# raynbowy23/RegT-GCN

Measured on AMD Instinct MI355X. Metric: training steps/sec (graph-snapshots/sec), higher is better.
Workload: dtype fp32; 1 GPU; cfg3: ONE synthetic regional graph, 100000 nodes / 1000000 edges / 8 regions, F=32, T=12, O=1, hidden=256; RegionalTemporalGCN forward+MSE+backward per snapshot, RMSprop step once per K steps (run.py semantics); gemm_arithmetic=fp32 MFMA (v_mfma_f32_32x32x2_f32), global_nodes=100000, global_edges=1000000, global_regions=8, parallelism=single GPU

## Files before the change

### regt-gcn_amd/csrc/gemm.hip

```cpp
#include "kernels.h"
#include "gemm_fast.h"
#include "gemm_split.h"
#include "gemm_small.h"

namespace regt {

#ifdef REGT_WG_TRACE
__device__ long g_wg_trace[4 * WG_TRACE_MAX];
__device__ long g_wg_marks[8 * WG_TRACE_MAX];
#define WG_TRACE_T(name) const long name = wall_clock64()
#define WG_TRACE_END(N, ta, tb)                                                                                              \
    if (threadIdx.x == 0 && WG_TILE_ID < WG_TRACE_MAX && (N) == REGT_WG_TRACE_N) {                                            \
        long* q_ = g_wg_trace + 4L * WG_TILE_ID;                                                                              \
        q_[0] = ta; q_[1] = tb; q_[2] = wall_clock64();                                                                       \
        q_[3] = ((long)__builtin_amdgcn_s_getreg((31 << 11) | 4)) | ((long)__builtin_amdgcn_s_getreg((31 << 11) | 20) << 32); \
    }
#else
#define WG_TRACE_T(name)
#define WG_TRACE_END(N, ta, tb)
#endif

__device__ __forceinline__ float fast_sigmoid(float x) { return __builtin_amdgcn_rcpf(1.0f + __expf(-x)); }
__device__ __forceinline__ float fast_tanh(float x) { return 1.0f - 2.0f * __builtin_amdgcn_rcpf(1.0f + __expf(2.0f * x)); }
__device__ __forceinline__ float4 ld4(const float* p) { return *reinterpret_cast<const float4*>(p); }
// ... 122 lines not shown
        long node = m / e.T;
        int t = (int)(m - node * e.T);
        float hv = e.h[m * e.C + c];
        float Z = e.ZR[m * (2L * e.C) + c];
        float R = e.ZR[m * (2L * e.C) + e.C + c];
        e.dzr[m * (2L * e.C) + e.C + c] = cb_drp(v, hv, R);
        e.dh[m * e.C + c] = cb_dh(v, R, e.probs[t], e.dOH[node * e.C + c], Z);
    }
    static constexpr int ROUND_ROWS = 8;
    struct Aux { float4 h, Z, R, d; float p; };
    __device__ __forceinline__ Aux load(long m, int c) const {
        const long node = m / e.T;
        Aux a;
        a.p = e.probs[(int)(m - node * e.T)];
        a.h = ld4(e.h + m * e.C + c);
        a.Z = ld4(e.ZR + m * (2L * e.C) + c);
        a.R = ld4(e.ZR + m * (2L * e.C) + e.C + c);
        a.d = ld4(e.dOH + node * e.C + c);
        return a;
    }
    __device__ __forceinline__ void apply(long m, int c, float4 v, const Aux& a) const {
#define F_(k) cb_drp(v.k, a.h.k, a.R.k)
        if (e.dzr_bf16) st4_bf16(e.dzr, m * (2L * e.C) + e.C + c, REGT_V4(F_));
        else st4(e.dzr + m * (2L * e.C) + e.C + c, REGT_V4(F_));
#undef F_
#define F_(k) cb_dh(v.k, a.R.k, a.p, a.d.k, a.Z.k)
        st4(e.dh + m * e.C + c, REGT_V4(F_));
#undef F_
    }
    static constexpr int NVAR = 2;
    static constexpr bool HAS_ROWTAB = true;
    struct Col {};
    struct Tile { __amdgpu_buffer_rsrc_t h, zr, d, dzr, dh; int vc, vzr, sc, szr, vd, vdzr, sdzr, rstep; const EpiRowEnt* rt; };
    __device__ __forceinline__ int variant(int) const { return e.dzr_bf16 ? 1 : 0; }
    __device__ __forceinline__ EpiRowEnt vrow(long m) const {
        const long node = m / e.T;
        return EpiRowEnt{(int)(node * e.C * 4), e.probs[(int)(m - node * e.T)]};
    }
    template <int V> __device__ __forceinline__ Col vcol(int) const { return Col{}; }
    template <int V> __device__ __forceinline__ Tile vtile(const EpiGeom& g) const {
        Tile t;
        t.h = buf_srd(e.h + g.m0 * e.C + g.n0);
        t.dh = buf_srd(e.dh + g.m0 * e.C + g.n0);
        t.zr = buf_srd(e.ZR + g.m0 * (2L * e.C) + g.n0);
        t.d = buf_srd(e.dOH + g.n0);
        const long o = g.m0 * (2L * e.C) + e.C + g.n0;
        t.dzr = buf_srd((V & 1) ? reinterpret_cast<const char*>(e.dzr) + 2 * o : reinterpret_cast<const char*>(e.dzr) + 4 * o);
        t.vc = (g.rr * e.C + g.c) * 4;
        t.sc = g.step * e.C * 4;
        t.vzr = 2 * t.vc - g.c * 4;
        t.szr = 2 * t.sc;
        t.vd = g.c * 4;
        t.vdzr = (V & 1) ? t.vzr >> 1 : t.vzr;
        t.sdzr = (V & 1) ? t.szr >> 1 : t.szr;
        t.rt = g.rowtab + g.rr;
        t.rstep = g.step;
        return t;
    }
    struct VAux { float4 h, Z, R, d; float p; };
    template <int V> __device__ __forceinline__ VAux vload(const Tile& t, int i) const {
        const EpiRowEnt re = t.rt[i * t.rstep];
        VAux a;
        a.p = re.p;
        a.h = buf_ld4(t.h, t.vc, i * t.sc);
        a.Z = buf_ld4(t.zr, t.vzr, i * t.szr);
        a.R = buf_ld4(t.zr, t.vzr, i * t.szr + e.C * 4);
        a.d = buf_ld4(t.d, t.vd + re.off, 0);
        return a;
    }
    template <int V> __device__ __forceinline__ void vapply(const Tile& t, int i, float4 v, const Col&, const VAux& a) const {
#define F_(k) cb_drp(v.k, a.h.k, a.R.k)
        if (V & 1) buf_st4_bf16(t.dzr, t.vdzr + i * t.sdzr, 0, REGT_V4(F_));
        else buf_st4(t.dzr, t.vdzr + i * t.sdzr, 0, REGT_V4(F_));
#undef F_
#define F_(k) cb_dh(v.k, a.R.k, a.p, a.d.k, a.Z.k)
        buf_st4(t.dh, t.vc + i * t.sc, 0, REGT_V4(F_));
#undef F_
    }
};
struct EpiDgrad1GenF {
    EpiDgrad1 e;
    int parts;
    static constexpr int ROUND_ROWS = 8;
    __device__ __forceinline__ static float half_wave_sum(float s) {
#define REGT_DPP_ADD(ctrl, rmask) s += __builtin_bit_cast(float, __builtin_amdgcn_update_dpp(0, __builtin_bit_cast(int, s), ctrl, rmask, 0xF, true))
        REGT_DPP_ADD(0xB1, 0xF);
        REGT_DPP_ADD(0x4E, 0xF);
        REGT_DPP_ADD(0x141, 0xF);
        REGT_DPP_ADD(0x140, 0xF);
        REGT_DPP_ADD(0x142, 0xA);
#undef REGT_DPP_ADD
        return s;
    }
    static constexpr int SUM_LANE = 31;
    static constexpr int EPI_AUX_BYTES = 192;
    struct Aux { float4 h, Z, R, d, t; float p; };
    __device__ __forceinline__ Aux load(long m, int c) const {
        const long node = m / e.T;
        Aux a;
        a.p = e.probs[(int)(m - node * e.T)];
        a.h = ld4(e.h + m * e.C + c);
        a.Z = ld4(e.ZR + m * (2L * e.C) + c);
        a.R = ld4(e.ZR + m * (2L * e.C) + e.C + c);
        a.d = ld4(e.dOH + node * e.C + c);
        a.t = ld4(e.Ht + m * e.C + c);
        return a;
    }
#define REGT_GEN_DOT(a) ((a.d.x * (a.Z.x * a.h.x + (1.0f - a.Z.x) * a.t.x) + a.d.y * (a.Z.y * a.h.y + (1.0f - a.Z.y) * a.t.y)) + \
                         (a.d.z * (a.Z.z * a.h.z + (1.0f - a.Z.z) * a.t.z) + a.d.w * (a.Z.w * a.h.w + (1.0f - a.Z.w) * a.t.w)))
    __device__ __forceinline__ void apply(long m, int c, float4 v, const Aux& a) const {
#define F_(k) cb_drp(v.k, a.h.k, a.R.k)
        st4(e.dzr + m * (2L * e.C) + e.C + c, REGT_V4(F_));
#undef F_
#define F_(k) cb_dh(v.k, a.R.k, a.p, a.d.k, a.Z.k)
        st4(e.dh + m * e.C + c, REGT_V4(F_));
#undef F_
#define F_(k) cb_dzp(__fmul_rn(a.p, a.d.k), a.h.k, a.t.k, a.Z.k)
        st4(e.dzr + m * (2L * e.C) + c, REGT_V4(F_));
#undef F_
        const float s = half_wave_sum(REGT_GEN_DOT(a));
        if ((threadIdx.x & 31) == SUM_LANE) e.rowdot[m * parts + c / GBN] = s;
    }
    static constexpr int NVAR = 1;
    static constexpr bool HAS_ROWTAB = true;
    struct Col {};
    struct Tile { __amdgpu_buffer_rsrc_t h, zr, d, dzr, dh, t, rd; int vc, vzr, sc, szr, vd, vrd, srd, rstep; const EpiRowEnt* rt; };
    __device__ __forceinline__ int variant(int) const { return 0; }
    __device__ __forceinline__ EpiRowEnt vrow(long m) const {
        const long node = m / e.T;
        return EpiRowEnt{(int)(node * e.C * 4), e.probs[(int)(m - node * e.T)]};
    }
    template <int V> __device__ __forceinline__ Col vcol(int) const { return Col{}; }
    template <int V> __device__ __forceinline__ Tile vtile(const EpiGeom& g) const {
        Tile t;
        t.h = buf_srd(e.h + g.m0 * e.C + g.n0);
        t.t = buf_srd(e.Ht + g.m0 * e.C + g.n0);
        t.dh = buf_srd(e.dh + g.m0 * e.C + g.n0);
        t.zr = buf_srd(e.ZR + g.m0 * (2L * e.C) + g.n0);
        t.d = buf_srd(e.dOH + g.n0);
        t.dzr = buf_srd(e.dzr + g.m0 * (2L * e.C) + g.n0);
        t.rd = buf_srd(e.rowdot + g.m0 * parts + g.n0 / GBN);
        t.vc = (g.rr * e.C + g.c) * 4;
        t.sc = g.step * e.C * 4;
        t.vzr = 2 * t.vc - g.c * 4;
        t.szr = 2 * t.sc;
        t.vd = g.c * 4;
        t.vrd = g.rr * parts * 4;
        t.srd = g.step * parts * 4;
        t.rt = g.rowtab + g.rr;
        t.rstep = g.step;
        return t;
    }
    struct VAux { float4 h, Z, R, d, t; float p; };
    template <int V> __device__ __forceinline__ VAux vload(const Tile& t, int i) const {
        const EpiRowEnt re = t.rt[i * t.rstep];
        VAux a;
        a.p = re.p;
        a.h = buf_ld4(t.h, t.vc, i * t.sc);
        a.Z = buf_ld4(t.zr, t.vzr, i * t.szr);
        a.R = buf_ld4(t.zr, t.vzr, i * t.szr + e.C * 4);
        a.d = buf_ld4(t.d, t.vd + re.off, 0);
        a.t = buf_ld4(t.t, t.vc, i * t.sc);
        return a;
    }
    template <int V> __device__ __forceinline__ void vapply(const Tile& t, int i, float4 v, const Col&, const VAux& a) const {
#define F_(k) cb_drp(v.k, a.h.k, a.R.k)
        buf_st4(t.dzr, t.vzr + i * t.szr + e.C * 4, 0, REGT_V4(F_));
#undef F_
#define F_(k) cb_dh(v.k, a.R.k, a.p, a.d.k, a.Z.k)
        buf_st4(t.dh, t.vc + i * t.sc, 0, REGT_V4(F_));
#undef F_
#define F_(k) cb_dzp(__fmul_rn(a.p, a.d.k), a.h.k, a.t.k, a.Z.k)
        buf_st4(t.dzr, t.vzr + i * t.szr, 0, REGT_V4(F_));
#undef F_
        const float s = half_wave_sum(REGT_GEN_DOT(a));
        if ((threadIdx.x & 31) == SUM_LANE) __builtin_amdgcn_raw_buffer_store_b32(__float_as_uint(s), t.rd, t.vrd + i * t.srd, 0, 0);
    }
#undef REGT_GEN_DOT
};
struct EpiDgrad2F {
    EpiDgrad2 e;
    __device__ __forceinline__ void operator()(long m, int c, float v) const {
        long i = m * e.C + c;
        float d = e.dh[i] + v;
        if (e.act == ACT_LRELU) d = e.h[i] > 0.f ? d : d * e.slope;
        e.dh[i] = d;
    }
    static constexpr int ROUND_ROWS = 16;
    struct Aux { float4 d, h; };
    __device__ __forceinline__ Aux load(long m, int c) const {
        Aux a;
        a.d = ld4(e.dh + m * e.C + c);
        a.h = e.act == ACT_LRELU ? ld4(e.h + m * e.C + c) : make_float4(1, 1, 1, 1);
        return a;
    }
    __device__ __forceinline__ void apply(long m, int c, float4 v, const Aux& a) const {
#define F_(k) ((a.d.k + v.k) * (a.h.k > 0.f ? 1.0f : e.slope))
        st4(e.dh + m * e.C + c, REGT_V4(F_));
#undef F_
    }
    static constexpr int NVAR = 2;
    static constexpr bool HAS_ROWTAB = false;
    struct Col {};
    struct VAux { float4 d, h; };
    struct Tile { __amdgpu_buffer_rsrc_t dh, h; int v, s; };
    __device__ __forceinline__ int variant(int) const { return e.act == ACT_LRELU ? 1 : 0; }
    template <int V> __device__ __forceinline__ Col vcol(int) const { return Col{}; }
    template <int V> __device__ __forceinline__ Tile vtile(const EpiGeom& g) const {
        Tile t;
        t.dh = buf_srd(e.dh + g.m0 * e.C + g.n0);
        if (V & 1) t.h = buf_srd(e.h + g.m0 * e.C + g.n0);
        t.v = (g.rr * e.C + g.c) * 4;
        t.s = g.step * e.C * 4;
        return t;
    }
    template <int V> __device__ __forceinline__ VAux vload(const Tile& t, int i) const {
        VAux a;
        a.d = buf_ld4(t.dh, t.v, i * t.s);
        if (V & 1) a.h = buf_ld4(t.h, t.v, i * t.s);
        return a;
    }
    template <int V> __device__ __forceinline__ void vapply(const Tile& t, int i, float4 v, const Col&, const VAux& a) const {
#define F_(k) ((a.d.k + v.k) * ((V & 1) ? (a.h.k > 0.f ? 1.0f : e.slope) : 1.0f))
        buf_st4(t.dh, t.v + i * t.s, 0, REGT_V4(F_));
#undef F_
    }
};
struct EpiMaskAddF {
    EpiMaskAdd e;
    __device__ __forceinline__ void operator()(long m, int c, float v) const {
        float o = e.mask[m * e.ldm + c] > 0.f ? v : 0.f;
        if (e.add) o += e.add[m * e.ldadd + c];
        e.out[m * e.ldo + c] = o;
    }
    static constexpr int ROUND_ROWS = 16;
    struct Aux { float4 mk, ad; };
    __device__ __forceinline__ Aux load(long m, int c) const {
        Aux a;
        a.mk = ld4(e.mask + m * e.ldm + c);
        a.ad = e.add ? ld4(e.add + m * e.ldadd + c) : make_float4(0, 0, 0, 0);
        return a;
    }
    __device__ __forceinline__ void apply(long m, int c, float4 v, const Aux& a) const {
#define F_(k) ((a.mk.k > 0.f ? v.k : 0.f) + a.ad.k)
        st4(e.out + m * e.ldo + c, REGT_V4(F_));
#undef F_
    }
    static constexpr int NVAR = 2;
    static constexpr bool HAS_ROWTAB = false;
    struct Col {};
    struct VAux { float4 mk, ad; };
    struct Tile { __amdgpu_buffer_rsrc_t out, mask, add; int vo, vm, va, so, sm, sa; };
    __device__ __forceinline__ int variant(int) const {
        return (e.ldo >= (1L << 22) || e.ldm >= (1L << 22) || (e.add && e.ldadd >= (1L << 22))) ? -1 : (e.add ? 1 : 0);
    }
    template <int V> __device__ __forceinline__ Col vcol(int) const { return Col{}; }
    template <int V> __device__ __forceinline__ Tile vtile(const EpiGeom& g) const {
        Tile t;
        t.out = buf_srd(e.out + g.m0 * e.ldo + g.n0);
        t.mask = buf_srd(e.mask + g.m0 * e.ldm + g.n0);
        if (V & 1) t.add = buf_srd(e.add + g.m0 * e.ldadd + g.n0);
// ... 300 lines not shown
    f32x16 acc[2][2];
#pragma unroll
    for (int i = 0; i < 2; ++i)
#pragma unroll
        for (int j = 0; j < 2; ++j)
#pragma unroll
            for (int r = 0; r < 16; ++r) acc[i][j][r] = 0.f;
    core.run(acc);
    if (vec) core.for_each_vec(acc, epi);
    else core.for_each(acc, [&](int r, int c, float v) { epi(m0 + r, c, v); });
}

template <class EpiF, class Core>
__global__ __launch_bounds__(256, 2) void gemm_flat_fast_kernel(GemmSegs S, long M, int N, EpiF epi, int relu_a) {
    extern __shared__ __attribute__((aligned(16))) float lds[];
    const int tiles_n = (N + GBN - 1) / GBN;
    const int bid = xcd_remap(blockIdx.x, gridDim.x);
    const long m0 = (long)(bid / tiles_n) * GBM;
    const int n0 = (bid % tiles_n) * GBN;
    RowMap rm{m0, 1, (int)((M - m0) < GBM ? (M - m0) : GBM)};
    Core core(S, rm, n0, N, lds);
    core.fill_rowtab(epi);
    core.plan();
    f32x16 acc[2][2];
#pragma unroll
    for (int i = 0; i < 2; ++i)
#pragma unroll
        for (int j = 0; j < 2; ++j)
#pragma unroll
            for (int r = 0; r < 16; ++r) acc[i][j][r] = 0.f;
    WG_TRACE_T(t_a);
    core.run(acc, relu_a != 0);
    WG_TRACE_T(t_b);
    core.for_each_vec(acc, epi);
    WG_TRACE_END(N, t_a, t_b);
}

template <class EpiF, bool REGION, int NP>
__global__ __launch_bounds__(256, 3) void gemm_flat_split_kernel(GemmSegs S, long M, int N, EpiF epi, int relu_a, int uniform) {
    extern __shared__ __attribute__((aligned(16))) float lds[];
    const int tiles_n = (N + GBN - 1) / GBN;
    const int bid = xcd_remap(blockIdx.x, gridDim.x);
    const long m0 = (long)(bid / tiles_n) * GBM;
    const int n0 = (bid % tiles_n) * GBN;
    RowMap rm{m0, 1, (int)((M - m0) < GBM ? (M - m0) : GBM)};
    WG_MARK(6);
    SplitCore<REGION, NP> core(S, rm, n0, N, lds, true);
    WG_MARK(7);
    core.fill_rowtab(epi);
    const bool uni = uniform != 0;
    if (!uni) core.plan();
    f32x16 acc[2][2];
#pragma unroll
    for (int i = 0; i < 2; ++i)
#pragma unroll
        for (int j = 0; j < 2; ++j)
#pragma unroll
            for (int r = 0; r < 16; ++r) acc[i][j][r] = 0.f;
    WG_TRACE_T(t_a);
    if (uni) core.run_uniform(acc, relu_a != 0);
    else core.run(acc, relu_a != 0);
    WG_TRACE_T(t_b);
    core.for_each_vec_halves(acc, epi);
    WG_TRACE_END(N, t_a, t_b);
}

template <int NP>
__global__ __launch_bounds__(256, 2) void gemm_dgrad1_gen_kernel(GemmSegs S, long M, int N, EpiDgrad1GenF epi) {
    extern __shared__ __attribute__((aligned(16))) float lds[];
    const int tiles_n = (N + GBN - 1) / GBN;
    const int bid = xcd_remap(blockIdx.x, gridDim.x);
    const long m0 = (long)(bid / tiles_n) * GBM;
    const int n0 = (bid % tiles_n) * GBN;
    RowMap rm{m0, 1, (int)((M - m0) < GBM ? (M - m0) : GBM)};
    SplitCore<false, NP> core(S, rm, n0, N, lds, true);
    core.fill_rowtab(epi);
    f32x16 acc[2][2];
#pragma unroll
    for (int i = 0; i < 2; ++i)
#pragma unroll
        for (int j = 0; j < 2; ++j)
#pragma unroll
            for (int r = 0; r < 16; ++r) acc[i][j][r] = 0.f;
    const typename SplitCore<false, NP>::AGen g{epi.e.ZR, epi.e.Ht, epi.e.dOH, epi.e.dhp, epi.e.C, (unsigned)epi.e.num_nodes * (unsigned)epi.e.C * 4u};
    core.run_u_gen(acc, g);
    core.for_each_vec_halves(acc, epi);
}

template <class EpiF8, bool REGION>
__global__ __launch_bounds__(256, 3) void gemm_flat_split8_kernel(GemmSegs S, long M, int N, EpiF8 epi, int uniform) {
    extern __shared__ __attribute__((aligned(16))) float lds[];
    const int tiles_n = (N + GBN - 1) / GBN;
    const int bid = xcd_remap(blockIdx.x, gridDim.x);
    const long m0 = (long)(bid / tiles_n) * GBM;
    const int n0 = (bid % tiles_n) * GBN;
    RowMap rm{m0, 1, (int)((M - m0) < GBM ? (M - m0) : GBM)};
    SplitCore<REGION, 1> core(S, rm, n0, N, lds, true);
    core.fill_rowtab(epi);
    const bool uni = uniform != 0;
    if (!uni) core.plan();
    f32x16 acc[2][2];
#pragma unroll
    for (int i = 0; i < 2; ++i)
#pragma unroll
        for (int j = 0; j < 2; ++j)
#pragma unroll
            for (int r = 0; r < 16; ++r) acc[i][j][r] = 0.f;
    WG_TRACE_T(t_a);
    if (uniform == 2) core.run_uniform_frag(acc, false);
    else if (uni) core.run_uniform(acc, false);
    else core.run(acc, false);
    WG_TRACE_T(t_b);
    core.for_each_vec8_halves(acc, epi);
    WG_TRACE_END(N, t_a, t_b);
}

template <class EpiF, bool BT, bool REGION>
__global__ __launch_bounds__(256, 4) void gemm_flat_small_kernel(GemmSegs S, long M, int N, EpiF epi, int relu_a) {
    extern __shared__ __attribute__((aligned(16))) float lds[];
    const int tiles_n = (N + SM_B - 1) / SM_B;
    const long m0 = (long)(blockIdx.x / tiles_n) * SM_B;
    const int n0 = (blockIdx.x % tiles_n) * SM_B;
    RowMap rm{m0, 1, (int)((M - m0) < SM_B ? (M - m0) : SM_B)};
    SmallCore<BT, REGION> core(S, rm, n0, N, lds);
    core.plan();
    f32x16 acc;
#pragma unroll
    for (int r = 0; r < 16; ++r) acc[r] = 0.f;
    core.run(acc, relu_a != 0);
    core.for_each_vec(acc, epi);
}

static thread_local int t_gemm_mode = -1;
int gemm_mode_override(int mode) { const int prev = t_gemm_mode; t_gemm_mode = mode; return prev; }
int gemm_mode() { return t_gemm_mode >= 0 ? t_gemm_mode : option(OPT_GEMM_MODE); }
bool fp32_core_wide() { return option(OPT_FP32_CORE) == 1; }

bool gemm_desc_table_forced() { return option(OPT_GEMM_DESC) == 1; }
static int uniform_ok(const GemmSegs& S, long M) {
    if (gemm_desc_table_forced()) return 0;
    int frag = 0;
    long slabs = 0;
    for (int s = 0; s < S.nseg; ++s) {
        const GemmSeg& g = S.seg[s];
        if (g.K % GBK != 0 || g.K <= 0) return 0;
        if ((g.flags & SEG_REGION) && (g.flags & SEG_A_BF16)) return 0;
        if (g.lda * 4 * (GBM + 1) >= (1L << 31) || g.ldb * 4 * (GBN + 1) >= (1L << 31)) return 0;
        if (g.flags & SEG_B_FRAG) ++frag;
        const long reps = (g.flags & SEG_REGION) ? std::min<long>(S.num_regions > 0 ? S.num_regions : 1, GBM / (S.row_div > 0 ? S.row_div : 1) + 2)
                                                 : ((g.flags & SEG_REPEAT) ? g.nrep : 1);
        slabs += reps * (g.K / GBK);
    }
    if (gemm_mode() == 2 && slabs > 64) return 0;
    (void)M;
    if (frag == 0) return 1;
    return frag == S.nseg && gemm_mode() == 2 ? 2 : 0;
}

static int fast_class(const GemmSegs& S, int N, bool vec) {
    if (!vec || N % 4 != 0 || S.nseg < 1) return -1;
    int bt = -1, region = 0, relu = 0;
    long iters = 0;
    for (int s = 0; s < S.nseg; ++s) {
        const GemmSeg& g = S.seg[s];
        if (!(g.flags & SEG_VEC_A) || !(g.flags & SEG_VEC_B) || g.K % 4 != 0) return -1;
        if ((g.flags & SEG_A_BF16) && (gemm_mode() != 2 || !(g.flags & SEG_BT) || g.K % 8 != 0 || g.lda % 8 != 0 ||
                                       (g.flags & (SEG_REGION | SEG_REPEAT | SEG_RELU_A)))) return -1;
// ... 855 lines not shown
```

### regt-gcn_amd/csrc/gemm_split.h

```cpp
#pragma once
#include <type_traits>
#include "gemm_fast.h"

namespace regt {

typedef __bf16 bf16x8 __attribute__((ext_vector_type(8)));
typedef __bf16 bf16x2 __attribute__((ext_vector_type(2)));
typedef float f32x2 __attribute__((ext_vector_type(2)));

constexpr int SP_ROW_B = 32;
constexpr int SP_PLANE_B = 128 * SP_ROW_B;
constexpr int CP_ROW_B = 64;
__device__ __forceinline__ constexpr int cp_off(int r, int g) { return r * CP_ROW_B + ((g ^ ((r >> 2) & 3)) << 4); }
template <int NP>
struct SplitGeom {
    static constexpr int OPER_B = NP == 0 ? 128 * CP_ROW_B : NP * SP_PLANE_B;
    static constexpr int STAGE_B = 2 * OPER_B;
    static constexpr int EPI_HALF_B = 64 * G_LDS_KROW * 4;
    static constexpr int TABLE_OFF_B = 2 * STAGE_B > EPI_HALF_B ? 2 * STAGE_B : EPI_HALF_B;
    static constexpr int LDS_BYTES = TABLE_OFF_B + G_TABLE_BYTES;
    static_assert(2 * STAGE_B <= 2 * G_STAGE * 4, "split stages fit the fp32 core's LDS footprint (table offset, epilogue image)");
};
constexpr int SP_LDS_BYTES = SplitGeom<3>::LDS_BYTES;
__device__ __forceinline__ constexpr int sp_off(int r, int g) { return r * SP_ROW_B + ((g ^ ((r >> 3) & 1)) << 4); }

template <class F> constexpr auto epi_aux_budget(int) -> decltype(F::EPI_AUX_BYTES) { return F::EPI_AUX_BYTES; }
template <class F> constexpr int epi_aux_budget(long) { return 96; }

template <bool REGION, int NP = 3>
struct SplitCore : FastCore<true, REGION> {
    using Base = FastCore<true, REGION>;
    using Geom = SplitGeom<NP>;
    static constexpr int OPER_B = Geom::OPER_B, STAGE_B = Geom::STAGE_B;
    using Srds = typename Base::Srds;
    using Base::S;
    using Base::rm;
    using Base::n0;
    using Base::N;
    using Base::lds;
    using Base::table;
    using Base::nit;
    using Base::tid;
    using Base::lane;
    using Base::wr;
    using Base::wc;
    int sreg[2];

    __device__ __forceinline__ SplitCore(const GemmSegs& s, RowMap r, int n0_, int N_, float* lds_, bool compact = false)
        : Base(s, r, n0_, N_, lds_) {
        if (compact) table = reinterpret_cast<ItDesc*>(reinterpret_cast<char*>(lds) + Geom::TABLE_OFF_B);
#pragma unroll
        for (int j = 0; j < 2; ++j) {
            const int rl = (tid >> 2) + 64 * j;
            sreg[j] = 0;
            if (REGION && rl < rm.nvalid) sreg[j] = S.node_region[rm.grow(rl) / S.row_div];
        }
    }

    __device__ __forceinline__ float4 sload_a(const Srds& d, int i) const {
        const int rl = (tid >> 2) + 64 * (i >> 1);
        const int k = d.k0 + 4 * ((tid & 3) + 4 * (i & 1));
        bool ok = rl < rm.nvalid && k < d.K;
        if (REGION) ok = ok && (d.region < 0 || sreg[i >> 1] == d.region);
        return Base::srd_load(d.a, ok ? 4u * (unsigned)(rl * (int)rm.mul * d.lda + k) : Base::SRD_OOB);
    }
    __device__ __forceinline__ float4 sload_b(const Srds& d, int i) const {
        const int nl = (tid >> 2) + 64 * (i >> 1);
        const int k = d.k0 + 4 * ((tid & 3) + 4 * (i & 1));
        const bool ok = n0 + nl < N && k < d.K;
        return Base::srd_load(d.b, ok ? 4u * (unsigned)(nl * d.ldb + k) : Base::SRD_OOB);
    }

    __device__ __forceinline__ static void split_store(char* q, float4 v, int plane_stride = SP_PLANE_B) {
        f32x2 lo = {v.x, v.y}, hi = {v.z, v.w};
#pragma unroll
        for (int p = 0; p < NP; ++p) {
            const bf16x2 bl = __builtin_convertvector(lo, bf16x2), bh = __builtin_convertvector(hi, bf16x2);
            const unsigned ul = __builtin_bit_cast(unsigned, bl), uh = __builtin_bit_cast(unsigned, bh);
            *reinterpret_cast<uint2*>(q + p * plane_stride) = make_uint2(ul, uh);
            if (p < NP - 1) {
                const f32x2 fl = {__uint_as_float(ul << 16), __uint_as_float(ul & 0xffff0000u)};
                const f32x2 fh = {__uint_as_float(uh << 16), __uint_as_float(uh & 0xffff0000u)};
                lo -= fl;
                hi -= fh;
            }
        }
    }
    template <bool RELU>
    __device__ __forceinline__ void store_half(int h, const float4 (&ra)[4], const float4 (&rb)[4], int abf = 0) const {
        char* st = reinterpret_cast<char*>(lds) + h * STAGE_B;
        if constexpr (NP == 0) {
#pragma unroll
            for (int j = 0; j < 2; ++j) {
                const int off = cp_off((tid >> 2) + 64 * j, tid & 3);
                float4 a = ra[h + 2 * j];
                if (RELU) { a.x = fmaxf(a.x, 0.f); a.y = fmaxf(a.y, 0.f); a.z = fmaxf(a.z, 0.f); a.w = fmaxf(a.w, 0.f); }
                *reinterpret_cast<float4*>(st + off) = a;
                *reinterpret_cast<float4*>(st + OPER_B + off) = rb[h + 2 * j];
            }
            return;
        }
        if (NP == 1 && abf) *reinterpret_cast<float4*>(st + sp_off(tid >> 1, tid & 1)) = ra[h];
#pragma unroll
        for (int j = 0; j < 2; ++j) {
            const int off = sp_off((tid >> 2) + 64 * j, (tid >> 1) & 1) + (tid & 1) * 8;
            if (!(NP == 1 && abf)) {
                float4 a = ra[h + 2 * j];
                if (RELU) { a.x = fmaxf(a.x, 0.f); a.y = fmaxf(a.y, 0.f); a.z = fmaxf(a.z, 0.f); a.w = fmaxf(a.w, 0.f); }
// ... 70 lines not shown
        if (NP == 1 && (g.flags & SEG_B_FRAG)) {
            d.bks = (g.K / 16) * 1024;
            const int nl = lowb ? n0 : n0 - g.nsplit;
            const char* bp = reinterpret_cast<const char*>(lowb ? g.B0 : g.B1) + boff + (long)(nl / 32) * d.bks;
            d.b = __builtin_amdgcn_make_buffer_rsrc(const_cast<char*>(bp), 0, live ? 4 * d.bks : 0, 0x00020000);
            d.vb[0] = 2 * wc * d.bks + lane * 16;
            d.vb[1] = 0;
            d.sb = (c.k0 / 16) * 1024;
        } else {
        const float* bp = lowb ? g.B0 + boff + (long)n0 * g.ldb : g.B1 + boff + (long)(n0 - g.nsplit) * g.ldb;
        const int blim = (lowb && g.nsplit < N ? g.nsplit : N) - n0, brows = blim < GBN ? blim : GBN;
        d.b = __builtin_amdgcn_make_buffer_rsrc(const_cast<float*>(bp), 0, live ? brows * ldb_b : 0, 0x00020000);
        d.vb[0] = (tid >> 2) * ldb_b + (tid & 3) * 16;
        d.vb[1] = d.vb[0] + 64 * ldb_b;
        d.sb = c.k0 * 4;
        }
        if (NP == 1 && d.abf) {
            d.va[0] = (tid >> 1) * lda_b + (tid & 1) * 16;
            d.va[1] = 0;
        } else {
            d.va[0] = (tid >> 2) * lda_b + (tid & 3) * 16;
            d.va[1] = d.va[0] + 64 * lda_b;
            if (REGION && reg) {
                d.va[0] = sreg[0] == region ? d.va[0] : (int)Base::SRD_OOB;
                d.va[1] = sreg[1] == region ? d.va[1] : (int)Base::SRD_OOB;
            }
        }
        d.sa = c.k0 * (d.abf ? 2 : 4);
        return d;
    }
    __device__ __forceinline__ void load_half(int h, const SrdsU& d, float4 (&ra)[4], float4 (&rb)[4]) const {
        if (NP == 1 && d.abf) {
            ra[h] = buf_ld4(d.a, d.va[0], d.sa + 32 * h);
        } else {
#pragma unroll
            for (int j = 0; j < 2; ++j) ra[h + 2 * j] = buf_ld4(d.a, d.va[j], d.sa + 64 * h);
        }
#pragma unroll
        for (int j = 0; j < 2; ++j) rb[h + 2 * j] = buf_ld4(d.b, d.vb[j], d.sb + 64 * h);
    }
    template <bool RELU>
    __device__ __forceinline__ void run_u(f32x16 (&acc)[2][2]) const {
        const int nslab = total_slabs();
        if (nslab == 0) return;
        float4 ra[4], rb[4];
        int held;
        SegCursor c{0, 0, 0};
        {
            const SrdsU d = make_u(c, true);
            load_half(0, d, ra, rb);
            load_half(1, d, ra, rb);
            held = d.abf;
        }
        store_half<RELU>(0, ra, rb, held);
        store_half<RELU>(1, ra, rb, held);
        {
            const bool two = nslab > 1;
            if (two) cursor_next(c);
            const SrdsU d = make_u(c, two);
            load_half(0, d, ra, rb);
            load_half(1, d, ra, rb);
            held = d.abf;
        }
        __syncthreads();
        compute(0, acc);
        for (int it = 0; it + 1 < nslab; ++it) {
            const bool live = it + 2 < nslab;
            if (live) cursor_next(c);
            const SrdsU nx = make_u(c, live);
            __syncthreads();
            fused<RELU>(0, 1, nx, ra, rb, acc, held);
            __syncthreads();
            fused<RELU>(1, 0, nx, ra, rb, acc, held);
            held = nx.abf;
        }
        __syncthreads();
        compute(1, acc);
        __syncthreads();
    }

    struct AGen {
        const float* ZR; const float* Ht; const float* dOH; float* dhp;
        int C; unsigned doh_bytes;
    };
    struct GenRegs { float4 z[4], t[4], d[4]; };
    struct GenRows { int vz[2], vh[2], vd[2]; float p[2]; };
    struct GenSrd { __amdgpu_buffer_rsrc_t z, t, d, o; };
    __device__ __forceinline__ GenRows gen_rows(const AGen& g) const {
        GenRows r;
#pragma unroll
        for (int j = 0; j < 2; ++j) {
            const int rl = (tid >> 2) + 64 * j;
            const EpiRowEnt re = Base::rowtab()[rl];
            r.p[j] = re.p;
            r.vd[j] = re.off + (tid & 3) * 16;
            r.vz[j] = rl * g.C * 8 + (tid & 3) * 16;
            r.vh[j] = rl * g.C * 4 + (tid & 3) * 16;
        }
        return r;
    }
    __device__ __forceinline__ GenSrd gen_srd(const AGen& g, bool live, bool writer) const {
        GenSrd s;
        const int C = g.C;
        s.z = __builtin_amdgcn_make_buffer_rsrc(const_cast<float*>(g.ZR + rm.base * 2L * C), 0, live ? rm.nvalid * C * 8 : 0, 0x00020000);
        s.t = __builtin_amdgcn_make_buffer_rsrc(const_cast<float*>(g.Ht + rm.base * (long)C), 0, live ? rm.nvalid * C * 4 : 0, 0x00020000);
        s.d = __builtin_amdgcn_make_buffer_rsrc(const_cast<float*>(g.dOH), 0, live ? (int)g.doh_bytes : 0, 0x00020000);
        s.o = __builtin_amdgcn_make_buffer_rsrc(g.dhp + rm.base * (long)C, 0, writer ? rm.nvalid * C * 4 : 0, 0x00020000);
        return s;
    }
    __device__ __forceinline__ void gen_load_half(int h, const GenSrd& s, const GenRows& r, int k0, GenRegs& q) const {
        const int so = (k0 + 16 * h) * 4;
#pragma unroll
        for (int j = 0; j < 2; ++j) {
            q.z[h + 2 * j] = buf_ld4(s.z, r.vz[j], so);
            q.t[h + 2 * j] = buf_ld4(s.t, r.vh[j], so);
            q.d[h + 2 * j] = buf_ld4(s.d, r.vd[j], so);
        }
    }
    __device__ __forceinline__ void gen_store_half(int h, const GenSrd& s, const GenRows& r, int k0, const GenRegs& q, const float4 (&rb)[4]) const {
        char* st = reinterpret_cast<char*>(lds) + h * STAGE_B;
        const int ko = (k0 + 16 * h) * 4;
#pragma unroll
        for (int j = 0; j < 2; ++j) {
            const int off = cp_off((tid >> 2) + 64 * j, tid & 3);
            const float4 z = q.z[h + 2 * j], t = q.t[h + 2 * j], d = q.d[h + 2 * j];
            const float p = r.p[j];
            float4 a;
            a.x = cb_dhp(__fmul_rn(p, d.x), z.x, t.x); a.y = cb_dhp(__fmul_rn(p, d.y), z.y, t.y);
            a.z = cb_dhp(__fmul_rn(p, d.z), z.z, t.z); a.w = cb_dhp(__fmul_rn(p, d.w), z.w, t.w);
            if constexpr (NP == 0) {
                *reinterpret_cast<float4*>(st + off) = a;
                *reinterpret_cast<float4*>(st + OPER_B + off) = rb[h + 2 * j];
            } else {
                const int offs = sp_off((tid >> 2) + 64 * j, (tid >> 1) & 1) + (tid & 1) * 8;
                asm volatile("" : "+v"(a.x), "+v"(a.y), "+v"(a.z), "+v"(a.w));
                split_store(st + offs, a);
                split_store(st + OPER_B + offs, rb[h + 2 * j]);
            }
            buf_st4(s.o, r.vh[j] + ko, 0, a);
        }
    }
    __device__ __forceinline__ void load_b_half(int h, const SrdsU& d, float4 (&rb)[4]) const {
#pragma unroll
        for (int j = 0; j < 2; ++j) rb[h + 2 * j] = buf_ld4(d.b, d.vb[j], d.sb + 64 * h);
    }
    __device__ __forceinline__ void run_u_gen(f32x16 (&acc)[2][2], const AGen& g) {
        static_assert(NP == 0 || NP == 3, "generated A operand: fp32 storage (fp32 MFMA or the exact bf16x3 split)");
        nreg_u = 0;
        const int nslab = S.seg[0].K / GBK;
        if (nslab == 0) return;
        const bool writer = n0 == 0;
        auto kof = [&](int i) { return i * GBK; };
        __syncthreads();
        const GenRows rows = gen_rows(g);
        GenRegs q;
        float4 rb[4];
        int k_held = kof(0);
        {
            const SrdsU d = make_u(SegCursor{0, 0, k_held}, true);
            const GenSrd s = gen_srd(g, true, writer);
            gen_load_half(0, s, rows, k_held, q);
            gen_load_half(1, s, rows, k_held, q);
            load_b_half(0, d, rb);
            load_b_half(1, d, rb);
            gen_store_half(0, s, rows, k_held, q, rb);
            gen_store_half(1, s, rows, k_held, q, rb);
        }
        {
            const bool two = nslab > 1;
            k_held = kof(two ? 1 : 0);
            const SrdsU d = make_u(SegCursor{0, 0, k_held}, two);
            const GenSrd s = gen_srd(g, two, writer);
            gen_load_half(0, s, rows, k_held, q);
            gen_load_half(1, s, rows, k_held, q);
            load_b_half(0, d, rb);
            load_b_half(1, d, rb);
        }
        __syncthreads();
        compute(0, acc);
        const GenSrd sw = gen_srd(g, true, writer);
        for (int it = 0; it + 1 < nslab; ++it) {
            const bool live = it + 2 < nslab;
            const int k_next = kof(live ? it + 2 : 0);
            const SrdsU nx = make_u(SegCursor{0, 0, k_next}, live);
            const GenSrd sn = gen_srd(g, live, writer);
            __syncthreads();
            fused_gen(0, 1, nx, sn, sw, rows, k_held, k_next, q, rb, acc);
            __syncthreads();
            fused_gen(1, 0, nx, sn, sw, rows, k_held, k_next, q, rb, acc);
            k_held = k_next;
        }
        __syncthreads();
        compute(1, acc);
        __syncthreads();
    }
    __device__ __forceinline__ void fused_gen(int hs, int hc, const SrdsU& nx, const GenSrd& sn, const GenSrd& sw, const GenRows& rows,
                                              int k_held, int k_next, GenRegs& q, float4 (&rb)[4], f32x16 (&acc)[2][2]) const {
        __builtin_amdgcn_sched_barrier(0);
        const Frags f = read_frags(hc);
        gen_store_half(hs, sw, rows, k_held, q, rb);
        mfmas(f, acc);
        gen_load_half(hs, sn, rows, k_next, q);
        load_b_half(hs, nx, rb);
        if constexpr (NP == 0) {
            __builtin_amdgcn_sched_group_barrier(0x100, 8, 0);
#pragma unroll
            for (int r = 0; r < 8; ++r) {
                __builtin_amdgcn_sched_group_barrier(0x008, 1, 0);
                __builtin_amdgcn_sched_group_barrier(0x006, 8, 0);
                if (r < 4) __builtin_amdgcn_sched_group_barrier(0x200, 1, 0);
                else __builtin_amdgcn_sched_group_barrier(0x020, 2, 0);
                if (r >= 2 && r < 4) __builtin_amdgcn_sched_group_barrier(0x040, 1, 0);
            }
        } else {
            __builtin_amdgcn_sched_group_barrier(0x100, 12, 0);
#pragma unroll
            for (int r = 0; r < 24; ++r) {
                __builtin_amdgcn_sched_group_barrier(0x008, 1, 0);
                __builtin_amdgcn_sched_group_barrier(0x002, 5, 0);
                if (r & 1) __builtin_amdgcn_sched_group_barrier(0x200, 1, 0);
                if (r >= 16) __builtin_amdgcn_sched_group_barrier(0x020, 1, 0);
                if (r >= 6 && r < 8) __builtin_amdgcn_sched_group_barrier(0x040, 1, 0);
            }
        }
        __builtin_amdgcn_sched_barrier(0);
    }

    struct FragsB { bf16x8 a[2][NP ? NP : 1], b[2][NP ? NP : 1]; };
    struct FragsF { float4 a[2][2], b[2][2]; };
    using Frags = std::conditional_t<NP == 0, FragsF, FragsB>;
    __device__ __forceinline__ Frags read_frags(int h) const {
        const char* st = reinterpret_cast<const char*>(lds) + h * STAGE_B;
        const int lr = lane & 31, lh = lane >> 5;
        Frags f;
        if constexpr (NP == 0) {
#pragma unroll
            for (int kk = 0; kk < 2; ++kk)
#pragma unroll
                for (int t = 0; t < 2; ++t) {
                    f.a[t][kk] = *reinterpret_cast<const float4*>(st + cp_off(wr * 64 + t * 32 + lr, 2 * kk + lh));
                    f.b[t][kk] = *reinterpret_cast<const float4*>(st + OPER_B + cp_off(wc * 64 + t * 32 + lr, 2 * kk + lh));
                }
            return f;
        } else {
#pragma unroll
        for (int p = NP - 1; p >= 0; --p)
#pragma unroll
            for (int t = 0; t < 2; ++t) {
                f.a[t][p] = *reinterpret_cast<const bf16x8*>(st + p * SP_PLANE_B + sp_off(wr * 64 + t * 32 + lr, lh));
                f.b[t][NP - 1 - p] = *reinterpret_cast<const bf16x8*>(st + OPER_B + (NP - 1 - p) * SP_PLANE_B + sp_off(wc * 64 + t * 32 + lr, lh));
            }
        return f;
        }
    }
    static constexpr int NPROD = NP == 3 ? 6 : 1;
    __device__ __forceinline__ static void mfmas(const Frags& f, f32x16 (&acc)[2][2]) {
        if constexpr (NP == 0) {
#pragma unroll
            for (int kk = 0; kk < 2; ++kk)
#pragma unroll
                for (int j = 0; j < 4; ++j)
#pragma unroll
                    for (int mt = 0; mt < 2; ++mt)
#pragma unroll
                        for (int nt = 0; nt < 2; ++nt)
                            acc[mt][nt] = __builtin_amdgcn_mfma_f32_32x32x2f32(reinterpret_cast<const float*>(&f.a[mt][kk])[j],
                                                                              reinterpret_cast<const float*>(&f.b[nt][kk])[j], acc[mt][nt], 0, 0, 0);
        } else {
        constexpr int PA[6] = {NP == 3 ? 2 : 0, 1, 0, 1, 0, 0}, PB[6] = {0, 1, 2, 0, 1, 0};
#pragma unroll
        for (int q = 0; q < NPROD; ++q)
#pragma unroll
            for (int mt = 0; mt < 2; ++mt)
#pragma unroll
                for (int nt = 0; nt < 2; ++nt)
                    acc[mt][nt] = __builtin_amdgcn_mfma_f32_32x32x16_bf16(f.a[mt][PA[q]], f.b[nt][PB[q]], acc[mt][nt], 0, 0, 0);
        }
    }
    __device__ __forceinline__ void compute(int h, f32x16 (&acc)[2][2]) const { mfmas(read_frags(h), acc); }

    __device__ __forceinline__ Frags read_frags_at(int stage) const {
        const char* st = reinterpret_cast<const char*>(lds) + stage * STAGE_B;
        const int lr = lane & 31, lh = lane >> 5;
        Frags f;
        if constexpr (NP == 1) {
#pragma unroll
            for (int t = 0; t < 2; ++t) {
                f.a[t][0] = *reinterpret_cast<const bf16x8*>(st + sp_off(wr * 64 + t * 32 + lr, lh));
                f.b[t][0] = *reinterpret_cast<const bf16x8*>(st + OPER_B + sp_off(wc * 64 + t * 32 + lr, lh));
            }
        }
        return f;
    }
    template <bool RELU>
    __device__ __forceinline__ void store_half_at(int stage, int h, const float4 (&ra)[4], const float4 (&rb)[4], int abf) const {
        char* st = reinterpret_cast<char*>(lds) + stage * STAGE_B;
        if (abf) *reinterpret_cast<float4*>(st + sp_off(tid >> 1, tid & 1)) = ra[h];
#pragma unroll
        for (int j = 0; j < 2; ++j) {
            const int off = sp_off((tid >> 2) + 64 * j, (tid >> 1) & 1) + (tid & 1) * 8;
            if (!abf) {
                float4 a = ra[h + 2 * j];
                if (RELU) { a.x = fmaxf(a.x, 0.f); a.y = fmaxf(a.y, 0.f); a.z = fmaxf(a.z, 0.f); a.w = fmaxf(a.w, 0.f); }
                split_store(st + off, a);
// ... 511 lines not shown
```

Measured before the change: 64.85 snapshots/s.

## Move dZ-gate and rowdot side outputs from dgrad1 epilogue into A-generation loop

```diff
diff --git a/regt-gcn_amd/csrc/gemm.hip b/regt-gcn_amd/csrc/gemm.hip
--- a/regt-gcn_amd/csrc/gemm.hip
+++ b/regt-gcn_amd/csrc/gemm.hip
@@ -228,19 +228,8 @@
     EpiDgrad1 e;
     int parts;
     static constexpr int ROUND_ROWS = 8;
-    __device__ __forceinline__ static float half_wave_sum(float s) {
-#define REGT_DPP_ADD(ctrl, rmask) s += __builtin_bit_cast(float, __builtin_amdgcn_update_dpp(0, __builtin_bit_cast(int, s), ctrl, rmask, 0xF, true))
-        REGT_DPP_ADD(0xB1, 0xF);
-        REGT_DPP_ADD(0x4E, 0xF);
-        REGT_DPP_ADD(0x141, 0xF);
-        REGT_DPP_ADD(0x140, 0xF);
-        REGT_DPP_ADD(0x142, 0xA);
-#undef REGT_DPP_ADD
-        return s;
-    }
-    static constexpr int SUM_LANE = 31;
-    static constexpr int EPI_AUX_BYTES = 192;
-    struct Aux { float4 h, Z, R, d, t; float p; };
+    static constexpr int EPI_AUX_BYTES = 136;
+    struct Aux { float4 h, Z, R, d; float p; };
     __device__ __forceinline__ Aux load(long m, int c) const {
         const long node = m / e.T;
         Aux a;
@@ -249,11 +238,8 @@
         a.Z = ld4(e.ZR + m * (2L * e.C) + c);
         a.R = ld4(e.ZR + m * (2L * e.C) + e.C + c);
         a.d = ld4(e.dOH + node * e.C + c);
-        a.t = ld4(e.Ht + m * e.C + c);
         return a;
     }
-#define REGT_GEN_DOT(a) ((a.d.x * (a.Z.x * a.h.x + (1.0f - a.Z.x) * a.t.x) + a.d.y * (a.Z.y * a.h.y + (1.0f - a.Z.y) * a.t.y)) + \
-                         (a.d.z * (a.Z.z * a.h.z + (1.0f - a.Z.z) * a.t.z) + a.d.w * (a.Z.w * a.h.w + (1.0f - a.Z.w) * a.t.w)))
     __device__ __forceinline__ void apply(long m, int c, float4 v, const Aux& a) const {
 #define F_(k) cb_drp(v.k, a.h.k, a.R.k)
         st4(e.dzr + m * (2L * e.C) + e.C + c, REGT_V4(F_));
@@ -261,16 +247,11 @@
 #define F_(k) cb_dh(v.k, a.R.k, a.p, a.d.k, a.Z.k)
         st4(e.dh + m * e.C + c, REGT_V4(F_));
 #undef F_
-#define F_(k) cb_dzp(__fmul_rn(a.p, a.d.k), a.h.k, a.t.k, a.Z.k)
-        st4(e.dzr + m * (2L * e.C) + c, REGT_V4(F_));
-#undef F_
-        const float s = half_wave_sum(REGT_GEN_DOT(a));
-        if ((threadIdx.x & 31) == SUM_LANE) e.rowdot[m * parts + c / GBN] = s;
     }
     static constexpr int NVAR = 1;
     static constexpr bool HAS_ROWTAB = true;
     struct Col {};
-    struct Tile { __amdgpu_buffer_rsrc_t h, zr, d, dzr, dh, t, rd; int vc, vzr, sc, szr, vd, vrd, srd, rstep; const EpiRowEnt* rt; };
+    struct Tile { __amdgpu_buffer_rsrc_t h, zr, d, dzr, dh; int vc, vzr, sc, szr, vd, rstep; const EpiRowEnt* rt; };
     __device__ __forceinline__ int variant(int) const { return 0; }
     __device__ __forceinline__ EpiRowEnt vrow(long m) const {
         const long node = m / e.T;
@@ -280,24 +261,20 @@
     template <int V> __device__ __forceinline__ Tile vtile(const EpiGeom& g) const {
         Tile t;
         t.h = buf_srd(e.h + g.m0 * e.C + g.n0);
-        t.t = buf_srd(e.Ht + g.m0 * e.C + g.n0);
         t.dh = buf_srd(e.dh + g.m0 * e.C + g.n0);
         t.zr = buf_srd(e.ZR + g.m0 * (2L * e.C) + g.n0);
         t.d = buf_srd(e.dOH + g.n0);
         t.dzr = buf_srd(e.dzr + g.m0 * (2L * e.C) + g.n0);
-        t.rd = buf_srd(e.rowdot + g.m0 * parts + g.n0 / GBN);
         t.vc = (g.rr * e.C + g.c) * 4;
         t.sc = g.step * e.C * 4;
         t.vzr = 2 * t.vc - g.c * 4;
         t.szr = 2 * t.sc;
         t.vd = g.c * 4;
-        t.vrd = g.rr * parts * 4;
-        t.srd = g.step * parts * 4;
         t.rt = g.rowtab + g.rr;
         t.rstep = g.step;
         return t;
     }
-    struct VAux { float4 h, Z, R, d, t; float p; };
+    struct VAux { float4 h, Z, R, d; float p; };
     template <int V> __device__ __forceinline__ VAux vload(const Tile& t, int i) const {
         const EpiRowEnt re = t.rt[i * t.rstep];
         VAux a;
@@ -306,7 +283,6 @@
         a.Z = buf_ld4(t.zr, t.vzr, i * t.szr);
         a.R = buf_ld4(t.zr, t.vzr, i * t.szr + e.C * 4);
         a.d = buf_ld4(t.d, t.vd + re.off, 0);
-        a.t = buf_ld4(t.t, t.vc, i * t.sc);
         return a;
     }
     template <int V> __device__ __forceinline__ void vapply(const Tile& t, int i, float4 v, const Col&, const VAux& a) const {
@@ -316,13 +292,7 @@
 #define F_(k) cb_dh(v.k, a.R.k, a.p, a.d.k, a.Z.k)
         buf_st4(t.dh, t.vc + i * t.sc, 0, REGT_V4(F_));
 #undef F_
-#define F_(k) cb_dzp(__fmul_rn(a.p, a.d.k), a.h.k, a.t.k, a.Z.k)
-        buf_st4(t.dzr, t.vzr + i * t.szr, 0, REGT_V4(F_));
-#undef F_
-        const float s = half_wave_sum(REGT_GEN_DOT(a));
-        if ((threadIdx.x & 31) == SUM_LANE) __builtin_amdgcn_raw_buffer_store_b32(__float_as_uint(s), t.rd, t.vrd + i * t.srd, 0, 0);
-    }
-#undef REGT_GEN_DOT
+    }
 };
 struct EpiDgrad2F {
     EpiDgrad2 e;
@@ -789,7 +759,8 @@
         for (int j = 0; j < 2; ++j)
 #pragma unroll
             for (int r = 0; r < 16; ++r) acc[i][j][r] = 0.f;
-    const typename SplitCore<false, NP>::AGen g{epi.e.ZR, epi.e.Ht, epi.e.dOH, epi.e.dhp, epi.e.C, (unsigned)epi.e.num_nodes * (unsigned)epi.e.C * 4u};
+    const typename SplitCore<false, NP>::AGen g{epi.e.ZR, epi.e.Ht, epi.e.dOH, epi.e.dhp, epi.e.C, (unsigned)epi.e.num_nodes * (unsigned)epi.e.C * 4u,
+                                                epi.e.h, epi.e.dzr, epi.e.rowdot, epi.parts};
     core.run_u_gen(acc, g);
     core.for_each_vec_halves(acc, epi);
 }
diff --git a/regt-gcn_amd/csrc/gemm_split.h b/regt-gcn_amd/csrc/gemm_split.h
--- a/regt-gcn_amd/csrc/gemm_split.h
+++ b/regt-gcn_amd/csrc/gemm_split.h
@@ -24,6 +24,8 @@
 constexpr int SP_LDS_BYTES = SplitGeom<3>::LDS_BYTES;
 __device__ __forceinline__ constexpr int sp_off(int r, int g) { return r * SP_ROW_B + ((g ^ ((r >> 3) & 1)) << 4); }
 
+#define REGT_GEN_DOT(a) ((a.d.x * (a.Z.x * a.h.x + (1.0f - a.Z.x) * a.t.x) + a.d.y * (a.Z.y * a.h.y + (1.0f - a.Z.y) * a.t.y)) + \
+                         (a.d.z * (a.Z.z * a.h.z + (1.0f - a.Z.z) * a.t.z) + a.d.w * (a.Z.w * a.h.w + (1.0f - a.Z.w) * a.t.w)))
 template <class F> constexpr auto epi_aux_budget(int) -> decltype(F::EPI_AUX_BYTES) { return F::EPI_AUX_BYTES; }
 template <class F> constexpr int epi_aux_budget(long) { return 96; }
 
@@ -260,10 +262,14 @@
     struct AGen {
         const float* ZR; const float* Ht; const float* dOH; float* dhp;
         int C; unsigned doh_bytes;
+        const float* h; float* dzr; float* rowdot; int parts;
     };
     struct GenRegs { float4 z[4], t[4], d[4]; };
     struct GenRows { int vz[2], vh[2], vd[2]; float p[2]; };
-    struct GenSrd { __amdgpu_buffer_rsrc_t z, t, d, o; };
+    struct GenSrd { __amdgpu_buffer_rsrc_t z, t, d; };
+    struct GenOut { __amdgpu_buffer_rsrc_t o, zo; };
+    struct GenDot { float4 d, Z, h, t; };
+    __device__ __forceinline__ bool owns(int k0) const { return k0 >= n0 && k0 < n0 + GBN; }
     __device__ __forceinline__ GenRows gen_rows(const AGen& g) const {
         GenRows r;
 #pragma unroll
@@ -277,14 +283,22 @@
         }
         return r;
     }
-    __device__ __forceinline__ GenSrd gen_srd(const AGen& g, bool live, bool writer) const {
+    __device__ __forceinline__ GenSrd gen_srd(const AGen& g, bool live) const {
         GenSrd s;
         const int C = g.C;
         s.z = __builtin_amdgcn_make_buffer_rsrc(const_cast<float*>(g.ZR + rm.base * 2L * C), 0, live ? rm.nvalid * C * 8 : 0, 0x00020000);
         s.t = __builtin_amdgcn_make_buffer_rsrc(const_cast<float*>(g.Ht + rm.base * (long)C), 0, live ? rm.nvalid * C * 4 : 0, 0x00020000);
         s.d = __builtin_amdgcn_make_buffer_rsrc(const_cast<float*>(g.dOH), 0, live ? (int)g.doh_bytes : 0, 0x00020000);
-        s.o = __builtin_amdgcn_make_buffer_rsrc(g.dhp + rm.base * (long)C, 0, writer ? rm.nvalid * C * 4 : 0, 0x00020000);
         return s;
+    }
+    __device__ __forceinline__ GenOut gen_out(const AGen& g, bool own) const {
+        GenOut s;
+        s.o = __builtin_amdgcn_make_buffer_rsrc(g.dhp + rm.base * (long)g.C, 0, own ? rm.nvalid * g.C * 4 : 0, 0x00020000);
+        s.zo = __builtin_amdgcn_make_buffer_rsrc(g.dzr + rm.base * 2L * g.C, 0, rm.nvalid * g.C * 8, 0x00020000);
+        return s;
+    }
+    __device__ __forceinline__ __amdgpu_buffer_rsrc_t gen_hsrd(const AGen& g, bool on) const {
+        return __builtin_amdgcn_make_buffer_rsrc(const_cast<float*>(g.h + rm.base * (long)g.C), 0, on ? rm.nvalid * g.C * 4 : 0, 0x00020000);
     }
     __device__ __forceinline__ void gen_load_half(int h, const GenSrd& s, const GenRows& r, int k0, GenRegs& q) const {
         const int so = (k0 + 16 * h) * 4;
@@ -295,7 +309,11 @@
             q.d[h + 2 * j] = buf_ld4(s.d, r.vd[j], so);
         }
     }
-    __device__ __forceinline__ void gen_store_half(int h, const GenSrd& s, const GenRows& r, int k0, const GenRegs& q, const float4 (&rb)[4]) const {
+    __device__ __forceinline__ void gen_load_h(int h, __amdgpu_buffer_rsrc_t s, const GenRows& r, int k0, float4 (&hq)[2]) const {
+#pragma unroll
+        for (int j = 0; j < 2; ++j) hq[j] = buf_ld4(s, r.vh[j], (k0 + 16 * h) * 4);
+    }
+    __device__ __forceinline__ void gen_store_half(int h, const GenOut& s, const GenRows& r, int k0, const GenRegs& q, const float4 (&rb)[4]) const {
         char* st = reinterpret_cast<char*>(lds) + h * STAGE_B;
         const int ko = (k0 + 16 * h) * 4;
 #pragma unroll
@@ -318,6 +336,19 @@
             buf_st4(s.o, r.vh[j] + ko, 0, a);
         }
     }
+    __device__ __forceinline__ void gen_side_half(int h, const GenOut& s, const GenRows& r, int k0, const GenRegs& q, const float4 (&hq)[2],
+                                                  float (&dot)[2]) const {
+        const int ko = (k0 + 16 * h) * 4;
+#pragma unroll
+        for (int j = 0; j < 2; ++j) {
+            const GenDot u{q.d[h + 2 * j], q.z[h + 2 * j], hq[j], q.t[h + 2 * j]};
+            const float p = r.p[j];
+#define F_(k) cb_dzp(__fmul_rn(p, u.d.k), u.h.k, u.t.k, u.Z.k)
+            buf_st4(s.zo, r.vz[j] + ko, 0, make_float4(F_(x), F_(y), F_(z), F_(w)));
+#undef F_
+            dot[j] += REGT_GEN_DOT(u);
+        }
+    }
     __device__ __forceinline__ void load_b_half(int h, const SrdsU& d, float4 (&rb)[4]) const {
 #pragma unroll
         for (int j = 0; j < 2; ++j) rb[h + 2 * j] = buf_ld4(d.b, d.vb[j], d.sb + 64 * h);
@@ -327,59 +358,84 @@
         nreg_u = 0;
         const int nslab = S.seg[0].K / GBK;
         if (nslab == 0) return;
-        const bool writer = n0 == 0;
         auto kof = [&](int i) { return i * GBK; };
         __syncthreads();
         const GenRows rows = gen_rows(g);
         GenRegs q;
-        float4 rb[4];
+        float4 rb[4], hq[2];
+        float dot[2] = {0.f, 0.f};
         int k_held = kof(0);
         {
+            const bool own = owns(k_held);
             const SrdsU d = make_u(SegCursor{0, 0, k_held}, true);
-            const GenSrd s = gen_srd(g, true, writer);
+            const GenSrd s = gen_srd(g, true);
+            const __amdgpu_buffer_rsrc_t sh = gen_hsrd(g, own);
+            float4 h0[2], h1[2];
+            gen_load_half(0, s, rows, k_held, q);
+            gen_load_h(0, sh, rows, k_held, h0);
+            gen_load_half(1, s, rows, k_held, q);
+            gen_load_h(1, sh, rows, k_held, h1);
+            load_b_half(0, d, rb);
+            load_b_half(1, d, rb);
+            const GenOut out = gen_out(g, own);
+            if (own) {
+                gen_side_half(0, out, rows, k_held, q, h0, dot);
+                gen_side_half(1, out, rows, k_held, q, h1, dot);
+            }
+            gen_store_half(0, out, rows, k_held, q, rb);
+            gen_store_half(1, out, rows, k_held, q, rb);
+        }
+        {
+            const bool two = nslab > 1;
+            k_held = kof(two ? 1 : 0);
+            const SrdsU d = make_u(SegCursor{0, 0, k_held}, two);
+            const GenSrd s = gen_srd(g, two);
             gen_load_half(0, s, rows, k_held, q);
             gen_load_half(1, s, rows, k_held, q);
             load_b_half(0, d, rb);
             load_b_half(1, d, rb);
-            gen_store_half(0, s, rows, k_held, q, rb);
-            gen_store_half(1, s, rows, k_held, q, rb);
-        }
-        {
-            const bool two = nslab > 1;
-            k_held = kof(two ? 1 : 0);
-            const SrdsU d = make_u(SegCursor{0, 0, k_held}, two);
-            const GenSrd s = gen_srd(g, two, writer);
-            gen_load_half(0, s, rows, k_held, q);
-            gen_load_half(1, s, rows, k_held, q);
-            load_b_half(0, d, rb);
-            load_b_half(1, d, rb);
+            gen_load_h(0, gen_hsrd(g, two && owns(k_held)), rows, k_held, hq);
         }
         __syncthreads();
         compute(0, acc);
-        const GenSrd sw = gen_srd(g, true, writer);
         for (int it = 0; it + 1 < nslab; ++it) {
             const bool live = it + 2 < nslab;
             const int k_next = kof(live ? it + 2 : 0);
             const SrdsU nx = make_u(SegCursor{0, 0, k_next}, live);
-            const GenSrd sn = gen_srd(g, live, writer);
-            __syncthreads();
-            fused_gen(0, 1, nx, sn, sw, rows, k_held, k_next, q, rb, acc);
-            __syncthreads();
-            fused_gen(1, 0, nx, sn, sw, rows, k_held, k_next, q, rb, acc);
+            const GenSrd sn = gen_srd(g, live);
+            const bool own = owns(k_held);
+            const __amdgpu_buffer_rsrc_t sh1 = gen_hsrd(g, own), sh0 = gen_hsrd(g, live && owns(k_next));
+            const GenOut out = gen_out(g, own);
+            __syncthreads();
+            if (own) gen_side_half(0, out, rows, k_held, q, hq, dot);
+            fused_gen(0, 1, nx, sn, out, sh1, 1, k_held, rows, k_held, k_next, q, rb, hq, acc);
+            __syncthreads();
+            if (own) gen_side_half(1, out, rows, k_held, q, hq, dot);
+            fused_gen(1, 0, nx, sn, out, sh0, 0, k_next, rows, k_held, k_next, q, rb, hq, acc);
             k_held = k_next;
         }
         __syncthreads();
         compute(1, acc);
-        __syncthreads();
-    }
-    __device__ __forceinline__ void fused_gen(int hs, int hc, const SrdsU& nx, const GenSrd& sn, const GenSrd& sw, const GenRows& rows,
-                                              int k_held, int k_next, GenRegs& q, float4 (&rb)[4], f32x16 (&acc)[2][2]) const {
+        const __amdgpu_buffer_rsrc_t rd = __builtin_amdgcn_make_buffer_rsrc(g.rowdot + rm.base * (long)g.parts + n0 / GBN, 0, rm.nvalid * g.parts * 4, 0x00020000);
+#pragma unroll
+        for (int j = 0; j < 2; ++j) {
+            float s = dot[j];
+            s += __builtin_bit_cast(float, __builtin_amdgcn_update_dpp(0, __builtin_bit_cast(int, s), 0xB1, 0xF, 0xF, true));
+            s += __builtin_bit_cast(float, __builtin_amdgcn_update_dpp(0, __builtin_bit_cast(int, s), 0x4E, 0xF, 0xF, true));
+            if ((tid & 3) == 0) __builtin_amdgcn_raw_buffer_store_b32(__float_as_uint(s), rd, ((tid >> 2) + 64 * j) * g.parts * 4, 0, 0);
+        }
+        __syncthreads();
+    }
+    __device__ __forceinline__ void fused_gen(int hs, int hc, const SrdsU& nx, const GenSrd& sn, const GenOut& out, __amdgpu_buffer_rsrc_t sh, int hh,
+                                              int k_h, const GenRows& rows, int k_held, int k_next, GenRegs& q, float4 (&rb)[4], float4 (&hq)[2],
+                                              f32x16 (&acc)[2][2]) const {
         __builtin_amdgcn_sched_barrier(0);
         const Frags f = read_frags(hc);
-        gen_store_half(hs, sw, rows, k_held, q, rb);
+        gen_store_half(hs, out, rows, k_held, q, rb);
         mfmas(f, acc);
         gen_load_half(hs, sn, rows, k_next, q);
         load_b_half(hs, nx, rb);
+        gen_load_h(hh, sh, rows, k_h, hq);
         if constexpr (NP == 0) {
             __builtin_amdgcn_sched_group_barrier(0x100, 8, 0);
 #pragma unroll
@@ -387,6 +443,7 @@
                 __builtin_amdgcn_sched_group_barrier(0x008, 1, 0);
                 __builtin_amdgcn_sched_group_barrier(0x006, 8, 0);
                 if (r < 4) __builtin_amdgcn_sched_group_barrier(0x200, 1, 0);
+                else if (r < 6) __builtin_amdgcn_sched_group_barrier(0x020, 3, 0);
                 else __builtin_amdgcn_sched_group_barrier(0x020, 2, 0);
                 if (r >= 2 && r < 4) __builtin_amdgcn_sched_group_barrier(0x040, 1, 0);
             }
@@ -397,7 +454,7 @@
                 __builtin_amdgcn_sched_group_barrier(0x008, 1, 0);
                 __builtin_amdgcn_sched_group_barrier(0x002, 5, 0);
                 if (r & 1) __builtin_amdgcn_sched_group_barrier(0x200, 1, 0);
-                if (r >= 16) __builtin_amdgcn_sched_group_barrier(0x020, 1, 0);
+                if (r >= 14) __builtin_amdgcn_sched_group_barrier(0x020, 1, 0);
                 if (r >= 6 && r < 8) __builtin_amdgcn_sched_group_barrier(0x040, 1, 0);
             }
         }
```

Result: slower. 63.30 snapshots/s (-2.4%).
